# nosnoc/LCQPow

Measured on AMD Instinct MI355X. Metric: LCQPs/sec (batched dense n=256,nC=512,nComp=64), higher is better.
Workload: dtype f64; 1 GPU; synthetic dense batch=1024/GPU n=256 nC=512 nComp=64 (BASELINE configs[2]; SplitMix64 seed0=0x4C43515000000001, perturbStep=0, printLevel=NONE); global_batch=1024, parallelism=batch-sharded x1, no collective, solved=1024

## Files before the change

include/lcqp_hip.h:

```cpp
#ifndef LCQP_HIP_H
#define LCQP_HIP_H

#include <stddef.h>
#include <stdint.h>

#ifdef __cplusplus
extern "C" {
#endif

#define LCQP_SUCCESSFUL_RETURN 0
#define LCQP_INVALID_ARGUMENT 100
#define LCQP_INVALID_OBJECTIVE_LINEAR_TERM 116
#define LCQP_INVALID_CONSTRAINT_MATRIX 117
#define LCQP_INVALID_COMPLEMENTARITY_MATRIX 118
#define LCQP_INVALID_LOWER_COMPLEMENTARITY_BOUND 120
#define LCQP_MAX_ITERATIONS_REACHED 200
#define LCQP_MAX_PENALTY_REACHED 201
#define LCQP_SUBPROBLEM_SOLVER_ERROR 203
#define LCQP_LCQPOBJECT_NOT_SETUP 300
#define LCQP_HIP_ERROR 900
#define LCQP_HIP_UNSUPPORTED 901

typedef struct {
    double complementarityTolerance;
// ... 106 lines not shown
                                           const double* R, const double* A, void* stream);
int  lcqp_hip_batch_get_solution_device(lcqp_hip_batch_t* b, double* x, double* y, lcqp_stats_t* stats, void* stream);
int  lcqp_hip_batch_sensitivity_device(lcqp_hip_batch_t* b, int blocked, int nrhs, const double* v,
                                       double* dg, double* db, int* side, int* info, void* stream);
int  lcqp_hip_batch_adjoint_device(lcqp_hip_batch_t* b, const double* vx, const double* vy,
                                   double* dg, double* db, int* side, int* info,
                                   int reduce, double* dQ, double* dA, double* dL, double* dR, void* stream);
int  lcqp_hip_batch_adjoint_blocked_device(lcqp_hip_batch_t* b, int nrhs, const double* vx, const double* vy,
                                           double* dg, double* db, int* side, int* info, void* stream);
int  lcqp_hip_batch_jacobian_device(lcqp_hip_batch_t* b, int first, int count, double* Jg, double* Jb, int* side, int* info, void* stream);
int  lcqp_hip_batch_jacobian_duals_device(lcqp_hip_batch_t* b, int first, int count, double* Jyg, double* Jyb, int* side, int* info, void* stream);

int  lcqp_hip_batch_get_trace(lcqp_hip_batch_t* b, int instance, int cap, double* scalars, double* x, int* len);
int  lcqp_hip_batch_read_profile(lcqp_hip_batch_t* b, unsigned long long* out);
void* lcqp_hip_batch_stream(lcqp_hip_batch_t* b);
double lcqp_hip_batch_algorithmic_bytes(lcqp_hip_batch_t* b);
int    lcqp_hip_batch_work_sums(lcqp_hip_batch_t* b, double out[6]);

int lcqp_hip_util_symv(int batch, int n, double alpha, const double* A, const double* b, const double* c, double* d);
int lcqp_hip_util_gemv_t(int batch, int m, int n, const double* A, const double* b, double* c);
int lcqp_hip_util_gemv(int batch, int m, int n, const double* A, const double* b, double* c);
int lcqp_hip_util_rows_list(int batch, int m, int n, const double* A, const int* list, int nlist, const double* x, const double* coef,
                            double* dots, double* outT);
int lcqp_hip_util_symm_product(int batch, int m, int n, const double* A, const double* B, double* C);
typedef struct lcqp_hip_csc lcqp_hip_csc_t;
lcqp_hip_csc_t* lcqp_hip_csc_create(int m, int n, int nnz, const int* p, const int* i, const double* x, int device);
void lcqp_hip_csc_destroy(lcqp_hip_csc_t* M);
int lcqp_hip_csc_apply(lcqp_hip_csc_t* M, int transposed, double alpha, const double* b, const double* c, double* d,
                       int repeat, float* ms);
int lcqp_hip_bench_rows(int batch, int m, int n, int mode, int repeat, float* ms);
int lcqp_hip_chol_solve(int batch, int n, const double* K, const double* b, double* x, int repeat, float* ms);


typedef struct lcqp_hip_sparse lcqp_hip_sparse_t;
lcqp_hip_sparse_t* lcqp_hip_sparse_create(int batch, int nV, int nC, int nComp, const int* Qp, const int* Qi,
                                          const int* Ap, const int* Ai, int device);
void lcqp_hip_sparse_destroy(lcqp_hip_sparse_t* s);
const char* lcqp_hip_sparse_last_error(void);
int  lcqp_hip_sparse_sched_profile(lcqp_hip_sparse_t* s, unsigned long long* out21);
int  lcqp_hip_sparse_bandwidth(const lcqp_hip_sparse_t* s);
int  lcqp_hip_sparse_lanes(const lcqp_hip_sparse_t* s);
int  lcqp_hip_sparse_fronts(const lcqp_hip_sparse_t* s);
int  lcqp_hip_sparse_general_ordering(const lcqp_hip_sparse_t* s);
int  lcqp_hip_sparse_border(const lcqp_hip_sparse_t* s);
int  lcqp_hip_sparse_get_ordering(const lcqp_hip_sparse_t* s, int* perm);
int  lcqp_hip_sparse_set_options(lcqp_hip_sparse_t* s, const lcqp_options_t* opt);
// ... 69 lines not shown
```

lcqpow_amd/__init__.py:

```python
from .capi import (Options, Stats, BatchLCQP, BatchPipeline, SubsolverHIP, default_options, lib, library_path, request_hw_queues, solve_mixed,
                   util_symv, util_gemv, util_gemv_t, util_symm_product, util_rows_list, chol_solve, device_count, CSCMatrix, SparseBatchLCQP,
                   split_bound_derivatives)
```

lcqpow_amd/capi.py:

```python
import contextlib
import ctypes as C
import os
import sys

import numpy as np

_HERE = os.path.dirname(os.path.abspath(__file__))
_SO = os.environ.get("LCQPOW_HIP_LIBRARY") or os.path.join(_HERE, "liblcqpow_hip.so")
c_double_p = C.POINTER(C.c_double)

SEED0 = 0x4C43515000000001
SUCCESSFUL_RETURN = 0
SUBPROBLEM_SOLVER_ERROR = 203
MAX_ITERATIONS_REACHED = 200
MAX_PENALTY_REACHED = 201


class Options(C.Structure):
    _fields_ = [
        ("complementarityTolerance", C.c_double), ("stationarityTolerance", C.c_double),
        ("initialPenaltyParameter", C.c_double), ("penaltyUpdateFactor", C.c_double),
        ("maxPenaltyParameter", C.c_double), ("etaDynamicPenalty", C.c_double),
        ("solveZeroPenaltyFirst", C.c_int), ("perturbStep", C.c_int), ("maxIterations", C.c_int),
        ("nDynamicPenalty", C.c_int), ("printLevel", C.c_int), ("storeSteps", C.c_int),
# ... 882 lines not shown
    _check(lib().lcqp_hip_util_gemv(batch, m, n, _p(A), _p(b), _p(c)), "util_gemv")
    return c


def util_gemv_t(A, b):
    A = _arr(A); b = _arr(b)
    batch, m, n = A.shape
    c = np.zeros((batch, n))
    _check(lib().lcqp_hip_util_gemv_t(batch, m, n, _p(A), _p(b), _p(c)), "util_gemv_t")
    return c


def util_rows_list(A, lists, x=None, coef=None, dots0=None):
    A = _arr(A); x = _arr(x); coef = _arr(coef)
    batch, m, n = A.shape
    lists = np.ascontiguousarray(lists, dtype=np.int32)
    dots = np.zeros((batch, m)) if dots0 is None else np.ascontiguousarray(dots0, dtype=np.float64).copy()
    out = np.zeros((batch, n))
    _check(lib().lcqp_hip_util_rows_list(batch, m, n, _p(A), lists.ctypes.data_as(C.POINTER(C.c_int)), lists.shape[1], _p(x), _p(coef),
                                         _p(dots) if x is not None else None, _p(out) if coef is not None else None), "util_rows_list")
    return dots, out


def util_symm_product(A, B):
    A = _arr(A); B = _arr(B)
    batch, m, n = A.shape
    Cm = np.zeros((batch, n, n))
    _check(lib().lcqp_hip_util_symm_product(batch, m, n, _p(A), _p(B), _p(Cm)), "util_symm_product")
    return Cm


def chol_solve(K, b, repeat=1):
    K = _arr(K); b = _arr(b)
    batch, n = K.shape[0], K.shape[1]
    x = np.zeros((batch, n)); ms = C.c_float(0)
    _check(lib().lcqp_hip_chol_solve(batch, n, _p(K), _p(b), _p(x), repeat, C.byref(ms)), "chol_solve")
    return x, ms.value


class CSCMatrix:

    def __init__(self, m, n, p, i, x, device=0):
        self.m, self.n = m, n
        p = np.ascontiguousarray(p, dtype=np.int32); i = np.ascontiguousarray(i, dtype=np.int32); x = _arr(x)
        ip = C.POINTER(C.c_int)
        self.h = lib().lcqp_hip_csc_create(m, n, len(x), p.ctypes.data_as(ip), i.ctypes.data_as(ip), _p(x), device)
# ... 207 lines not shown
```

lcqpow_amd/csrc/lcqp_dev.hpp:

```cpp
#pragma once
#include "lcqp_wg.hpp"
#include "../../include/lcqp_hip.h"

namespace lcqp {

enum { V_G, V_GPHI, V_GTIL, V_XK, V_PK, V_XNEW, V_GK, V_QX, V_CX, V_QP, V_CP, V_STATK, V_TMP,
       V_XQ, V_XA, V_XT, V_R1, V_C, V_DU, V_W, V_RHS, V_LB, V_UB, V_X0, V_R1S, V_GS, V_ATY, V_QXN, V_XS, V_XREF, V_NUM };
enum { M_L, M_U, M_RHOV, M_YQ, M_YA, M_ZA, M_YT, M_EX, M_COEF, M_EXS, M_DY, M_RN, M_MG, M_YLV, M_HOTV, M_NUM };
enum { I_ST, I_STT, I_DEP, I_PRIO, I_SLOT, I_LIST, I_LIST2, I_HOTC, I_NUM };
enum { S_R2, S_DY, S_D0, S_SV, S_W, S_NUM };

struct InstInfo {
    int mE, nfin, hasY0, setupFail, haveSolution, isSetup, nT, prioCtr;
    int ndep, ns;
    int cNnz, kReady, rnReady, nHot;
    double scale, sigma, spv, rhoAdmm, phiConst;
    int warm, pad0;
    double rho0;
    double hist[64];
    double work[6];
};

struct DevBatch {
    int B, n, np, nC, nComp, mA, boxcap, mEcap, capS, nblk, nd;
// ... 49 lines not shown
    c.E = db.E + (size_t)b * db.mEcap * np; c.Et = db.Et + (size_t)b * db.mEcap * np;
    c.F1 = db.F1 + (size_t)b * np * np; c.FK = db.FK + (size_t)b * np * np;
    c.S = db.S + (size_t)b * db.capS * db.capS;
    c.MM = db.MM + (size_t)b * db.mMld * db.mMld;
    c.S2 = db.S2 + (size_t)b * db.capS * db.capS; c.DS = db.DS + (size_t)b * (db.capS / 64) * 4096;
    c.crow = db.crow + (size_t)b * db.capS;
    c.D1 = db.D1 + (size_t)b * db.nblk * 4096; c.dscr = db.dscr + (size_t)b * 4096;
    c.nv = db.nv + (size_t)b * V_NUM * np; c.mv = db.mv + (size_t)b * M_NUM * db.mEcap;
    c.sv = db.sv + (size_t)b * S_NUM * db.capS;
    c.mi = db.mi + (size_t)b * I_NUM * db.mEcap; c.idx = db.idx + (size_t)b * db.capS;
    c.boxidx = db.boxidx + (size_t)b * np;
    c.info = db.info + b;
    c.mE = uniform_i(c.info->mE);
    c.lds = lds;
    c.cAdmm = c.cTrials = c.cFact = c.cCorr = c.cSweeps = 0;
#ifdef LCQP_PROFILE
    for (int k = 0; k < 16; k++) c.prof[k] = 0;
    c.tlast = clock64();
#endif
    return c;
}

enum { P_LCQP = 0, P_RESID = 1, P_GRAM = 2, P_CHOL = 3, P_CORR_L1 = 4, P_CORR_ROWS = 5, P_CORR_S = 6, P_ADMM = 7, P_MISC = 8, P_DEL = 9, P_UPD_PRE = 10 };
#if defined(LCQP_PROFILE) && !defined(LCQP_PROFILE_BULK)
#define PROF(c, k) do { unsigned long long t_ = clock64(); (c).prof[k] += t_ - (c).tlast; (c).tlast = t_; } while (0)
#else
#define PROF(c, k) do { } while (0)
#endif
#if defined(LCQP_PROFILE) && defined(LCQP_PROFILE_BULK)
#define PROFB0(c) do { (c).tlast = clock64(); } while (0)
#define PROFB(c, k) do { unsigned long long t_ = clock64(); (c).prof[k] += t_ - (c).tlast; (c).tlast = t_; } while (0)
#else
#define PROFB0(c) do { } while (0)
#define PROFB(c, k) do { } while (0)
#endif

__device__ __forceinline__ double clipd(double v, double lo, double hi) { return v < lo ? lo : (v > hi ? hi : v); }

template <int NCH>
__device__ __forceinline__ void qp_admm(Ctx<NCH>& c, const double* g, int n_it)
{
    constexpr int np = 128 * NCH;
    const lcqp_options_t& o = c.db->opt;
    const int t = tid_here(), mE = c.mE;
    const double alpha = o.admmAlpha, sigma = c.info->sigma;
    double *xa = c.V(V_XA), *rhs = c.V(V_RHS), *w = c.V(V_W);
    double *ya = c.M(M_YA), *za = c.M(M_ZA), *rhov = c.M(M_RHOV), *coef = c.M(M_COEF), *ex = c.M(M_EX), *dyl = c.M(M_DY);
    const double *l = c.M(M_L), *u = c.M(M_U);
    PROF(c, P_MISC);
    for (int it = 0; it < n_it; it++) {
        const int t = tid_here();
        for (int r = t; r < mE; r += WG) coef[r] = rhov[r] * za[r] - ya[r];
        __syncthreads();
        wg_rows<NCH>(c.E, nullptr, mE, nullptr, nullptr, coef, c.lds,
                     [&](int i, double s) { rhs[i] = sigma * xa[i] - g[i] + s; });
        wg_trsv<wg_ncopy(NCH) == 2>(c.FK, np, c.nblk, rhs, true, c.lds);
        wg_trsv<wg_ncopy(NCH) == 2>(c.FK, np, c.nblk, rhs, false, c.lds);
// ... 546 lines not shown
    int* hotc = c.I(I_HOTC);
    const double* hotv = c.M(M_HOTV);
    const double *l = c.M(M_L), *u = c.M(M_U);
    int *dep = c.I(I_DEP), *prio = c.I(I_PRIO), *list = c.I(I_LIST), *rslot = c.I(I_SLOT);
    double *r2 = c.Sv(S_R2), *dy = c.Sv(S_DY);
    int* idx = c.idx;
    const double shrinkF = uniform_d(1.0 + 1e-6 + o.feasTol);
    int na = 0, nsl = 0, fact_valid = 0;
    int prioCtr = uniform_i(c.info->prioCtr);
    const int capNa = min(min(min(max(2 * c.n, 64), mE), capS), max_active(NCH));

    double xnrm = 0.0;
    int capOn = 0;
    int nrefine = 0;
    const int maxTrials = damp ? o.maxTrials + 4 * c.n + 32 : o.maxTrials;
    const PolishView v = {x, r1, cv, du, qx, xs, xref, yt, ex, mg, st, ylv, rn, hotc, hotv, l, u, dep, prio, list, rslot, r2, dy, idx,
                          g, ytol, rtolG, reuse, damp, spv, shrinkF, capNa, maxTrials};
    for (int trial = 0; trial < maxTrials; trial++) {
        const int t = tid_here();
        c.cTrials++;
        int changed = 0, nlv = 0, have_true = 0, need_true = 0;
        const bool cold = (trial == 0 && !reuse);
        PROF(c, P_MISC);
        if (trial == 0) {
            if (reuse) {
                const double *r1s = c.V(V_R1S), *gs0 = c.V(V_GS), *exs = c.M(M_EXS);
                for (int i = t; i < np; i += WG) r1[i] = (r1s[i] + (gs0[i] - g[i])) - spv * (x[i] - xref[i]);
                wg_map<4>(mE, [&](int r) { return exs[r]; }, [&](int r, double v) { ex[r] = v; });
                __syncthreads();
                have_true = 1;
            } else {
                if (!uniform_i(c.info->rnReady)) {
                    wg_row_norms<NCH>(c.E, mE, rn, hotc, c.M(M_HOTV));
                    int nh = 0;
                    for (int r = t; r < mE; r += WG) nh += (hotc[r] >= 0);
                    nh = block_sum_i(nh, c.lds);
                    if (t == 0) { c.info->rnReady = 1; c.info->nHot = nh; }
                }
                int cntA = 0;
                wg_map<4>(mE, [&](int r) { return MapID{st[r], yt[r]}; },
                          [&](int r, MapID v) { if (v.s == ST_INACT && v.a != 0.0) yt[r] = 0.0; ylv[r] = 0.0; cntA += (v.s != ST_INACT); });
                capOn = (block_sum_i(cntA, c.lds) == 0);
                (void)polish_sweep_distance<NCH>(c, v, xnrm);
                need_true = 1;
            }
        } else {
            const double dl = polish_sweep_distance<NCH>(c, v, xnrm);
            int cntLv = 0;
            int rLeave = -1;
            if (damp) rLeave = polish_damped_leave_row(st, yt, mE, ytol, t, c.lds);
            wg_map<4>(mE, [&](int r) { return MapID3{st[r], yt[r], mg[r], rn[r]}; },
                      [&](int r, MapID3 v) {
                          int s = v.s;
                          if (((s == ST_LOWER && v.a > ytol) || (s == ST_UPPER && v.a < -ytol)) && (!damp || r == rLeave)) { ylv[r] = v.a; yt[r] = 0.0; st[r] = ST_INACT; s = ST_INACT; cntLv++; }
                          mg[r] = (s != ST_INACT) ? -1.0 : v.b - v.c * dl;
                      });
            nlv = block_sum_i(cntLv, c.lds);
            changed = nlv > 0;
            const bool depRows = uniform_i(c.info->ndep) > 0;
            const int nread = wg_compact(mE, [&](int r) { return (st[r] == ST_INACT) ? !(mg[r] > 1e-10) : (depRows && dep[r] != 0); }, list, c.lds);
            wg_rows<NCH, true>(c.E, list, nread, x, ex, nullptr, c.lds, [](int, double) {}, hotc, hotv);
            double vcut = 0.0;
            int rEnter = -1;
            if (damp) {
                vcut = INFINITY;
                if (!changed) {
                    double vm = 0.0;
                    for (int a = t; a < nread; a += WG) vm = fmax(vm, polish_violation(v, o, list[a]));
                    vm = block_max(vm, c.lds);
                    if (vm > 0.0) {
                        int rb = 1 << 30;
                        for (int a = t; a < nread; a += WG) { const int r = list[a]; if (polish_violation(v, o, r) >= vm) rb = min(rb, r); }
                        rEnter = (int)(-block_max((double)(-rb), c.lds) + 0.5);
                        vcut = vm;
                    }
                }
            } else
            if (capOn) {
                double vm = 0.0, cv = 0.0, vmax, nviol;
                for (int a = t; a < nread; a += WG) { const double vi = polish_violation(v, o, list[a]); if (vi > 0.0) { cv += 1.0; vm = fmax(vm, vi); } }
                block_max_sum(vm, cv, vmax, nviol, c.lds);
                const int cap = max(c.n / 8, 16);
                if (nviol > (double)cap) {
                    double lo = 0.0, hi = vmax;
// ... 14 lines not shown
                const double e = ex[r], ftol = o.feasTol * (1.0 + fabs(e));
                if (s == ST_INACT) {
                    const bool may = !damp || r == rEnter;
                    if (may && e < l[r] - ftol && l[r] - e >= vcut) { st[r] = ST_LOWER; chg |= 1; }
                    else if (may && e > u[r] + ftol && e - u[r] >= vcut) { st[r] = ST_UPPER; chg |= 1; }
                    else mg[r] = fmin(e - (l[r] - ftol), (u[r] + ftol) - e);
                } else if (depRows && dep[r]) {
                    bool viol, inside = false;
                    if (s == ST_LOWER) { viol = e < l[r] - ftol; inside = e > l[r] + ftol; }
                    else if (s == ST_UPPER) { viol = e > u[r] + ftol; inside = e < u[r] - ftol; }
                    else viol = fabs(e - l[r]) > ftol;
                    if (inside) { const double yv = yt[r]; ylv[r] = yv; yt[r] = 0.0; st[r] = ST_INACT; cntLv2 += (yv != 0.0); chg |= 1; }
                    else if (viol) { prio[r] = prioCtr + 1; chg |= 2; }
                }
            }
            if (depRows) nlv += block_sum_i(cntLv2, c.lds);
            const bool countDense = mE <= 4000;
            const unsigned packed = (unsigned)block_sum_i((chg & 1) | (((chg >> 1) & 1) << 10) | ((countDense ? nDense : 0) << 20), c.lds);
            const int chgBits = ((packed & 1023u) ? 1 : 0) | (((packed >> 10) & 1023u) ? 2 : 0);
            if (t == 0) c.info->work[4] += countDense ? (double)(packed >> 20) : (double)nread;
            if (chgBits & 2) { prioCtr++; if (t == 0) c.info->prioCtr = prioCtr; }
            changed |= (chgBits != 0);
            need_true = !changed;
        }
        PROF(c, P_RESID);
        if (need_true) {
            int* lact = c.I(I_LIST2);
            wg_symv<NCH>(c.Q, nullptr, c.n, x, nullptr, qx, nullptr, nullptr, nullptr, c.lds);
            const int nact = wg_compact(mE, [&](int r) { return cold || st[r] != ST_INACT; }, lact, c.lds);
            wg_rows<NCH, true>(c.E, lact, nact, x, ex, yt, c.lds, [&](int i, double s) { const double ro = -g[i] - qx[i] - s; du[i] = ro; r1[i] = ro - spv * (x[i] - xref[i]); cv[i] = fabs(g[i]) + fabs(qx[i]) + fabs(s); }, hotc, hotv);
            c.cSweeps++;
            if (cold) {
                if (t == 0) c.info->work[4] += (double)(nact - uniform_i(c.info->nHot));
                wg_map<4>(mE, [&](int r) { return MapID3{st[r], ex[r], l[r], u[r]}; },
                          [&](int r, MapID3 v) {
                              const double e = v.a, ftol = o.feasTol * (1.0 + fabs(e));
                              mg[r] = (v.s != ST_INACT) ? -1.0 : fmin(e - (v.b - ftol), (v.c + ftol) - e);
                          });
                __syncthreads();
            } else {
                double res_stat, rscale;
                wg_maxabs2(r1, cv, np, c.n, res_stat, rscale, c.lds);
                const double rtolS = uniform_d(fmax(rtolG, 64.0 * 2.221e-16 * rscale));
                double res_eq = 0.0, bmax = 0.0, nDense2 = 0.0;
                for (int a = t; a < nact; a += WG) {
                    const int r = lact[a];
                    const int s = st[r];
                    nDense2 += (hotc[r] < 0) ? 1.0 : 0.0;
                    if (s == ST_INACT) continue;
                    const double bb = (s == ST_UPPER) ? u[r] : l[r];
                    const double rr = fabs(bb - ex[r]);
                    const bool above = rr > 16.0 * 2.221e-16 * (fabs(bb) + rn[r] * xnrm);
                    if (above) res_eq = fmax(res_eq, rr);
                    bmax = fmax(bmax, fabs(bb));
                    if (rslot[r] >= 0 && above) nDense2 += 1048576.0;
                }
                int nloose;
                { double re, nd; block_max_sum(res_eq, nDense2, re, nd, c.lds); res_eq = re; nloose = (int)(nd * (1.0 / 1048576.0)); nd -= 1048576.0 * nloose; if (t == 0) c.info->work[4] += nd; }
                bmax = block_max(bmax, c.lds);
#ifdef LCQP_TRACE_QP
                if (tid_here() == 0) printf("  hip trial %d stage 2: res_stat %.3e (tol %.3e) res_eq %.3e (tol %.3e) loose %d scale %.2e |x| %.2e\n", trial, res_stat, rtolS, res_eq, o.resTol * (1.0 + bmax), nloose, rscale, xnrm);
#endif
                if (res_stat <= rtolS && res_eq <= o.resTol * (1.0 + bmax) && nloose > 0 && nrefine < 2 && trial + 1 < maxTrials) {
                    nrefine++;
                } else
                if (res_stat <= rtolS && res_eq <= o.resTol * (1.0 + bmax) && !(wg_maxabs(du, np, c.lds) <= rtolS)) {
                    for (int i = t; i < np; i += WG) { xref[i] = x[i]; r1[i] = du[i]; }
                    __syncthreads();
                } else
                if (res_stat <= rtolS && res_eq <= o.resTol * (1.0 + bmax)) {
                    double *r1s = c.V(V_R1S), *gs0 = c.V(V_GS), *exs = c.M(M_EXS), *aty = c.V(V_ATY);
                    double* qxn = c.V(V_QXN);
                    for (int i = t; i < np; i += WG) { const double ro = du[i]; r1s[i] = ro; gs0[i] = g[i]; aty[i] = g[i] + qx[i] + ro; qxn[i] = qx[i]; }
                    wg_map<4>(mE, [&](int r) { return ex[r]; }, [&](int r, double v) { exs[r] = v; });
                    __syncthreads();
                    PROF(c, P_RESID);
                    return 1;
                }
            }
            have_true = 1;
            PROF(c, P_RESID);
        }
        if (changed) fact_valid = 0;
        if (!fact_valid) {
            int nT = uniform_i(c.info->nT), ns = uniform_i(c.info->ns);
            int touched = 0, ndepNow = 0;
            const int ndel = wg_compact(ns, [&](int sl) { const int r = idx[sl]; return r >= 0 && st[r] == ST_INACT; }, list, c.lds);
            int cntAdd = 0;
            wg_map<4>(mE, [&](int r) { return MapID{st[r], (double)rslot[r]}; }, [&](int, MapID v) { cntAdd += (v.s != ST_INACT && v.a < 0.0); });
            const int nadd = block_sum_i(cntAdd, c.lds);
            if (trial >= 2 && nT - ndel + nadd > c.n && ndel + nadd > max(c.n / 2, 32)) { polish_give_up<NCH>(c, v); return 0; }
            PROF(c, P_UPD_PRE);
            const bool bulk = prioCtr > 0 || (nT == 0 && nadd > 0) || (ndel > 0 && ndel >= max(nT / 2, 8)) || nadd >= 16 || (3 * ndel + 7 * nadd >= 96);
            int naAll = 0;
            if (bulk) {
                int cntAct = 0;
                for (int r = t; r < mE; r += WG) cntAct += (st[r] != ST_INACT);
                naAll = block_sum_i(cntAct, c.lds);
                ti_reset<NCH>(c, nT, ns);
            }
            if (bulk && naAll <= capNa) {
                int na2 = 0;
                for (int stamp = prioCtr; stamp >= 1; stamp--)
                    na2 += wg_compact(mE, [&](int r) { return st[r] != ST_INACT && prio[r] == stamp; }, idx + na2, c.lds);
// ... 501 lines not shown
```

lcqpow_amd/csrc/lcqp_hip_util.hip:

```cpp
#include "lcqp_hip_batch.hpp"
#include "../../include/lcqp_synth.h"

#include <algorithm>
#include <cstring>
#include <memory>
#include <vector>

using namespace lcqp;
using namespace lcqp_rt;

__global__ __launch_bounds__(WG) void k_chol(int np, int nblk, int n, double* F, double* dscr, int* fail)
{
    LCQP_LDS
    const int b = blockIdx.x;
    wg_chol(F + (size_t)b * np * np, np, nblk, n, 0.0, dscr + (size_t)b * 4096, nullptr, fail + b, lds, 0);
}

__global__ __launch_bounds__(WG, 4) void k_backsolve(int np, int nblk, const double* F, const double* rhs, double* x)
{
    LCQP_LDS
    const int b = blockIdx.x;
    double* xv = x + (size_t)b * np;
    for (int i = threadIdx.x; i < np; i += WG) xv[i] = rhs[(size_t)b * np + i];
    __syncthreads();
// ... 79 lines not shown

extern "C" int lcqp_hip_util_rows_list(int batch, int m, int n, const double* A, const int* list, int nlist, const double* x, const double* coef,
                                       double* dots, double* outT)
{ return guarded(dense_err(), [&] {
    if (n <= 0 || n > 4096 || batch <= 0 || m <= 0 || nlist < 0 || nlist > m || !list) return LCQP_HIP_UNSUPPORTED;
    const SizeKernels* k = dense_kernels(padded_nch(n));
    if (!k) return LCQP_HIP_UNSUPPORTED;
    const int np = 128 * k->nch;
    DevMem tb;
    double *dA, *dx = nullptr, *dd = nullptr, *dcf = nullptr, *dout = nullptr;
    int* dl;
    if (!tb.alloc(dense_err(), dA, (size_t)batch * m * np) || (x && !tb.alloc(dense_err(), dx, (size_t)batch * np)) ||
        (dots && !tb.alloc(dense_err(), dd, (size_t)batch * m, dots)) ||
        (coef && !tb.alloc(dense_err(), dcf, (size_t)batch * m, coef)) || (outT && !tb.alloc(dense_err(), dout, (size_t)batch * np)) ||
        !tb.alloc(dense_err(), dl, (size_t)batch * nlist, list))
        return LCQP_HIP_ERROR;
    int rc = upload_padded(dA, A, batch, m, n, np, m); if (rc) return rc;
    if (x) { rc = upload_padded(dx, x, batch, 1, n, np, 1); if (rc) return rc; }
    k->util_rows_list(batch, 0, m, nlist, dA, dl, dx, dd, dcf, dout);
    HIPCHK(dense_err(), hipDeviceSynchronize());
    if (dots) HIPCHK(dense_err(), hipMemcpy(dots, dd, sizeof(double) * (size_t)batch * m, hipMemcpyDeviceToHost));
    if (outT) return download_padded(outT, dout, batch, 1, n, np, 1);
    return 0;
}); }

extern "C" int lcqp_hip_util_gemv(int batch, int m, int n, const double* A, const double* b, double* c)
{
    return guarded(dense_err(), [&] { return util_rows(batch, m, n, A, b, c, nullptr, nullptr); });
}
extern "C" int lcqp_hip_util_gemv_t(int batch, int m, int n, const double* A, const double* b, double* c)
{
    return guarded(dense_err(), [&] { return util_rows(batch, m, n, A, nullptr, nullptr, b, c); });
}

extern "C" int lcqp_hip_util_symm_product(int batch, int m, int n, const double* A, const double* Bm, double* C)
{ return guarded(dense_err(), [&] {
    lcqp_hip_batch* h = lcqp_hip_batch_create(batch, n, 0, m, 0, 0);
    if (!h) return LCQP_HIP_ERROR;
    DevBatch& d = h->db;
    int rc = upload_padded(d.E, A, batch, m, n, d.np, d.mEcap);
    if (!rc) {
        std::vector<double> buf((size_t)d.mEcap * d.np);
        for (int b = 0; b < batch && !rc; b++) {
            if (hipMemcpy(buf.data(), d.E + (size_t)b * d.mEcap * d.np, sizeof(double) * buf.size(), hipMemcpyDeviceToHost) != hipSuccess) { rc = LCQP_HIP_ERROR; break; }
            for (int r = 0; r < m; r++) memcpy(&buf[(size_t)(m + r) * d.np], Bm + ((size_t)b * m + r) * n, sizeof(double) * n);
            if (hipMemcpy(d.E + (size_t)b * d.mEcap * d.np, buf.data(), sizeof(double) * buf.size(), hipMemcpyHostToDevice) != hipSuccess) rc = LCQP_HIP_ERROR;
// ... 194 lines not shown
```

lcqpow_amd/csrc/lcqp_kernels.hpp:

```cpp
#pragma once
#include "lcqp_dev.hpp"
#include "lcqp_launch.hpp"
#include "../../include/lcqp_synth.h"

using namespace lcqp;


template <int NCH>
__device__ __forceinline__ double prepare_vectors(const DevBatch& db, Ctx<NCH>& c, Lds lds, double scale)
{
    constexpr int np = 128 * NCH;
    const int b = c.b, t = threadIdx.x;
    const int mA = db.mA, nC = db.nC, nComp = db.nComp;
    const int nfin = c.info->nfin;
    const int mE = mA + nfin;
    double *l = c.M(M_L), *u = c.M(M_U), *rhov = c.M(M_RHOV);
    for (int k = t; k < nfin; k += WG) {
        const int bi = c.boxidx[k];
        l[mA + k] = c.V(V_LB)[bi]; u[mA + k] = c.V(V_UB)[bi];
    }
    __syncthreads();
    const double rho = db.opt.admmRho * scale;
    for (int r = t; r < mE; r += WG) {
        const double lo = l[r], hi = u[r];
// ... 1083 lines not shown
template <int NCH>
__global__ __launch_bounds__(WG) void k_util_rows(int m, const double* A, const double* x, double* dots, const double* coef, double* outT)
{
    LCQP_LDS_N(NCH)
    constexpr int np = 128 * NCH;
    const int b = blockIdx.x;
    double* o = outT ? outT + (size_t)b * np : nullptr;
    wg_rows<NCH>(A + (size_t)b * m * np, nullptr, m, x ? x + (size_t)b * np : nullptr, dots ? dots + (size_t)b * m : nullptr,
                 coef ? coef + (size_t)b * m : nullptr, lds, [&](int i, double s) { if (o) o[i] = s; });
}

template <int NCH>
__global__ __launch_bounds__(WG) void k_util_rows_list(int m, int nlist, const double* A, const int* list, const double* x, double* dots, const double* coef, double* outT)
{
    LCQP_LDS_N(NCH)
    constexpr int np = 128 * NCH;
    const int b = blockIdx.x;
    double* o = outT ? outT + (size_t)b * np : nullptr;
    wg_rows<NCH, true>(A + (size_t)b * m * np, list + (size_t)b * nlist, nlist, x ? x + (size_t)b * np : nullptr, dots ? dots + (size_t)b * m : nullptr,
                       coef ? coef + (size_t)b * m : nullptr, lds, [&](int i, double s) { if (o) o[i] = s; });
}

template <int NCH>
static void launch_run(const DevBatch& db, int grid, hipStream_t s)
{
    if constexpr (NCH <= 2) {
        static_assert(6 * 128 * NCH <= LDS_ROWS_OFF, "k_lcqp_run<NCH, true>: the sweeps' scratch must end below the row state");
        if (db.mEcap <= LDS_ROWS_MAX && 4 * db.capS <= LDS_ROWS_OFF) { hipLaunchKernelGGL((k_lcqp_run<NCH, true, LCQP_VARIANT>), dim3(grid), dim3(WG), 0, s, db); return; }
    }
    hipLaunchKernelGGL((k_lcqp_run<NCH, false, LCQP_VARIANT>), dim3(grid), dim3(WG), 0, s, db);
}

template <int NCH>
static void launch_qp_solve(const DevBatch& db, int grid, hipStream_t s, int initial)
{
    hipLaunchKernelGGL((k_qp_solve<NCH, LCQP_VARIANT>), dim3(grid), dim3(WG), 0, s, db, initial);
}

namespace lcqp {
#ifdef LCQP_TU_FEW
template <int NCH>
const RunKernels& few_kernels()
{
    static const RunKernels k = {launch_run<NCH>, launch_qp_solve<NCH>};
    return k;
}
// ... 23 lines not shown
        };
        t.sensitivity_dual = [](const DevBatch& db, int grid, hipStream_t s, int nrhs, const double* v, const double* vy, double* dg, double* dbo, int* side, int* sinfo) {
            hipLaunchKernelGGL((k_sensitivity<NCH, true>), dim3(grid), dim3(WG), 0, s, db, nrhs, v, dg, dbo, side, sinfo, vy);
        };
        t.build_C = [](const DevBatch& db, int grid, hipStream_t s) { hipLaunchKernelGGL((k_build_C<NCH>), dim3(grid), dim3(WG), 0, s, db); };
        t.compress_C = [](const DevBatch& db, int grid, hipStream_t s) { hipLaunchKernelGGL((k_compress_C<NCH>), dim3(grid), dim3(WG), 0, s, db); };
        t.factor = [](const DevBatch& db, int grid, hipStream_t s) { hipLaunchKernelGGL((k_factor<NCH, 1>), dim3(grid), dim3(WG), 0, s, db); };
        t.factor_full = [](const DevBatch& db, int grid, hipStream_t s) { hipLaunchKernelGGL((k_factor<NCH, NCH <= 2 ? 4 : 1>), dim3(grid), dim3(WG), 0, s, db); };
        t.trsm = [](const DevBatch& db, int grid, hipStream_t s) { hipLaunchKernelGGL((k_trsm<NCH>), dim3(grid), dim3(WG), 0, s, db); };
        t.trsm_streamed = [](const DevBatch& db, int grid, hipStream_t s) { hipLaunchKernelGGL((k_trsm_streamed<NCH>), dim3(grid), dim3(WG), 0, s, db); };
        t.build_M = [](const DevBatch& db, int grid, hipStream_t s) { hipLaunchKernelGGL((k_build_M<NCH>), dim3(grid), dim3(WG), 0, s, db); };
        t.run = {launch_run<NCH>, launch_qp_solve<NCH>};
        t.synth_fill = [](const DevBatch& db, int grid, hipStream_t s, uint64_t seed0, uint64_t first) { hipLaunchKernelGGL((k_synth_fill<NCH>), dim3(grid), dim3(WG), 0, s, db, seed0, first); };
        t.synth_Q = [](const DevBatch& db, int grid, hipStream_t s) { hipLaunchKernelGGL((k_synth_Q<NCH>), dim3(grid), dim3(WG), 0, s, db); };
        t.util_symv = [](int grid, hipStream_t s, int n, double alpha, const double* A, const double* b, const double* c, double* d) {
            hipLaunchKernelGGL((k_util_symv<NCH>), dim3(grid), dim3(WG), 0, s, n, alpha, A, b, c, d);
        };
        t.util_rows = [](int grid, hipStream_t s, int m, const double* A, const double* x, double* dots, const double* coef, double* outT) {
            hipLaunchKernelGGL((k_util_rows<NCH>), dim3(grid), dim3(WG), 0, s, m, A, x, dots, coef, outT);
        };
        t.util_rows_list = [](int grid, hipStream_t s, int m, int nlist, const double* A, const int* list, const double* x, double* dots, const double* coef, double* outT) {
            hipLaunchKernelGGL((k_util_rows_list<NCH>), dim3(grid), dim3(WG), 0, s, m, nlist, A, list, x, dots, coef, outT);
        };
        return t;
    }();
    return k;
}
#endif
}
```

lcqpow_amd/csrc/lcqp_launch.hpp:

```cpp
#pragma once
#include "lcqp_dev.hpp"

namespace lcqp {
#pragma GCC visibility push(hidden)

struct RunKernels {
    void (*lcqp_run)(const DevBatch& db, int grid, hipStream_t s);
    void (*qp_solve)(const DevBatch& db, int grid, hipStream_t s, int initial);
};

using BatchKernel = void (*)(const DevBatch& db, int grid, hipStream_t s);

struct SizeKernels {
    int nch;
    RunKernels run;
    const RunKernels* few;
    BatchKernel prepare;
    void (*refresh)(const DevBatch& db, int grid, hipStream_t s, int mode, const double* rho0);
    void (*prepare_warm)(const DevBatch& db, int grid, hipStream_t s, const double* rho0);
    BatchKernel build_C, compress_C;
    BatchKernel factor, factor_full;
    BatchKernel trsm, trsm_streamed, build_M;
    void (*synth_fill)(const DevBatch& db, int grid, hipStream_t s, uint64_t seed0, uint64_t first);
    BatchKernel synth_Q;
    void (*sensitivity)(const DevBatch& db, int grid, hipStream_t s, int nrhs, const double* v, double* dg, double* dbo, int* side, int* sinfo);
    void (*sensitivity_dual)(const DevBatch& db, int grid, hipStream_t s, int nrhs, const double* v, const double* vy, double* dg, double* dbo, int* side, int* sinfo);
    void (*sensitivity_blk)(const DevBatch& db, int grid, hipStream_t s, int first, int nrhs, const double* v, double* dg, double* dbo, int* side, int* sinfo);
    void (*sensitivity_blk_dual)(const DevBatch& db, int grid, hipStream_t s, int first, int nrhs, const double* v, const double* vy, int unit,
                                 double* dg, double* dbo, int* side, int* sinfo, int* rowpos);
    void (*util_symv)(int grid, hipStream_t s, int n, double alpha, const double* A, const double* b, const double* c, double* d);
    void (*util_rows)(int grid, hipStream_t s, int m, const double* A, const double* x, double* dots, const double* coef, double* outT);
    void (*util_rows_list)(int grid, hipStream_t s, int m, int nlist, const double* A, const int* list, const double* x, double* dots, const double* coef, double* outT);
};

template <int NCH> const SizeKernels& size_kernels();
template <int NCH> const RunKernels& few_kernels();

#pragma GCC visibility pop
}
```

lcqpow_amd/csrc/lcqp_wg.hpp:

```cpp
#pragma once
#include <hip/hip_runtime.h>
#include <stdint.h>

namespace lcqp {

constexpr int WG = 256;
constexpr int NWAVE = 4;
constexpr int wg_ncopy(int nch) { return nch > 16 ? 2 : 4; }
constexpr int arena_doubles(int nch) { return (wg_ncopy(nch) + 2) * 128 * nch > 4512 ? (wg_ncopy(nch) + 2) * 128 * nch : 4512; }
constexpr int ARENA = arena_doubles(4);
constexpr int TILE_LD = 65;
constexpr int max_active(int nch) { return 64 * (arena_doubles(nch) / (5 * 64)); }
constexpr int LCQP_MAX_ACTIVE = max_active(4);

enum { ST_INACT = 0, ST_LOWER = 1, ST_UPPER = 2, ST_EQ = 3 };

constexpr int LDS_ROWS_MAX = 640;
constexpr int LDS_ROWS_OFF = 2048;
static_assert(LDS_ROWS_OFF + 3 * LDS_ROWS_MAX + LDS_ROWS_MAX / 2 <= 4512, "row state must fit the arena");

struct Lds {
    double* arena;
    double* red;
    int* ired;
// ... 382 lines not shown
                }
            }
#pragma unroll
            for (int d = 0; d < D; d++) {
                if (x) {
                    double dsum = 0.0;
#pragma unroll
                    for (int k = 0; k < NCH; k++) dsum += mm[d][k].x * xr[2 * k] + mm[d][k].y * xr[2 * k + 1];
                    dsum = wave_sum(dsum);
                    if (l == j0 + d) mydot = dsum;
                }
                if (coef && cfs[d] != 0.0) {
#pragma unroll
                    for (int k = 0; k < NCH; k++) { acc[2 * k] += cfs[d] * mm[d][k].x; acc[2 * k + 1] += cfs[d] * mm[d][k].y; }
                }
            }
        }
        if (mine && dots && (!BYROW || myrow >= 0)) dots[BYROW ? myrow : mya] = mydot;
    }
    if (coef) wg_combine<NCH>(acc, lds, post);
    else __syncthreads();
}

template <bool TWO = false>
__device__ __forceinline__ void wg_trsv(const double* __restrict__ F, int ld, int nblk, double* vec, bool forward, Lds lds)
{
    const int nn = 64 * nblk;
    double* b = lds.arena;
    double* red = lds.arena + nn;
    for (int i = tid_here(); i < nn; i += WG) b[i] = vec[i];
    __syncthreads();
    const int l = lane_id(), w = wave_id();
    for (int s = 0; s < nblk; s++) {
        const int I = forward ? s : nblk - 1 - s;
        {
            const double* Fd = F + (size_t)(64 * I) * ld + 64 * I;
            double f[16];
#pragma unroll
            for (int cc = 0; cc < 16; cc++) {
                const int c = 16 * w + cc;
                f[cc] = 0.0;
                if (forward ? (c <= l) : (c >= l)) f[cc] = ld_stream(Fd + (size_t)c * ld + l);
            }
            double acc = 0.0;
#pragma unroll
            for (int cc = 0; cc < 16; cc++) {
// ... 350 lines not shown
```

Baseline: 31010 LCQPs/s.

## Fuse Q symv with active-row E products in the residual stage

Adds a fused device routine that streams Q rows and the active E rows in one pass, producing Qx, E^T y and the row dots together with one shared LDS reduction instead of separate symv and row passes. It is used for small padded sizes (NCH<=2, which covers n=256), while larger sizes keep the old two-call path. The leaving-row check is also switched to a dots-only routine that skips the combine reduction. A test utility and residual-stage profiling macros are added as well. This trades extra registers and a larger LDS footprint (eight partial copies) for fewer barriers and passes.

```diff
diff --git a/include/lcqp_hip.h b/include/lcqp_hip.h
--- a/include/lcqp_hip.h
+++ b/include/lcqp_hip.h
@@ -152,6 +152,8 @@
 int lcqp_hip_util_gemv(int batch, int m, int n, const double* A, const double* b, double* c);
 int lcqp_hip_util_rows_list(int batch, int m, int n, const double* A, const int* list, int nlist, const double* x, const double* coef,
                             double* dots, double* outT);
+int lcqp_hip_util_symv_rows(int batch, int n, int m, const double* Q, const double* E, const int* list, int nlist, const double* x, const double* coef,
+                            int use_hot, int two_pass, double* qx, double* ety, double* dots);
 int lcqp_hip_util_symm_product(int batch, int m, int n, const double* A, const double* B, double* C);
 typedef struct lcqp_hip_csc lcqp_hip_csc_t;
 lcqp_hip_csc_t* lcqp_hip_csc_create(int m, int n, int nnz, const int* p, const int* i, const double* x, int device);
diff --git a/lcqpow_amd/__init__.py b/lcqpow_amd/__init__.py
--- a/lcqpow_amd/__init__.py
+++ b/lcqpow_amd/__init__.py
@@ -1,3 +1,3 @@
 from .capi import (Options, Stats, BatchLCQP, BatchPipeline, SubsolverHIP, default_options, lib, library_path, request_hw_queues, solve_mixed,
-                   util_symv, util_gemv, util_gemv_t, util_symm_product, util_rows_list, chol_solve, device_count, CSCMatrix, SparseBatchLCQP,
+                   util_symv, util_gemv, util_gemv_t, util_symm_product, util_rows_list, util_symv_rows, chol_solve, device_count, CSCMatrix, SparseBatchLCQP,
                    split_bound_derivatives)
diff --git a/lcqpow_amd/capi.py b/lcqpow_amd/capi.py
--- a/lcqpow_amd/capi.py
+++ b/lcqpow_amd/capi.py
@@ -928,6 +928,19 @@
     return dots, out
 
 
+def util_symv_rows(Q, E, lists, x, coef, use_hot=False, two_pass=False, dots0=None):
+    Q = _arr(Q); E = _arr(E); x = _arr(x); coef = _arr(coef)
+    batch, m, n = E.shape
+    lists = np.ascontiguousarray(lists, dtype=np.int32).reshape(batch, -1)
+    dots = np.zeros((batch, m)) if dots0 is None else np.ascontiguousarray(dots0, dtype=np.float64).copy()
+    qx, ety = np.zeros((batch, n)), np.zeros((batch, n))
+    f = lib().lcqp_hip_util_symv_rows
+    f.argtypes = [C.c_int, C.c_int, C.c_int, c_double_p, c_double_p, C.POINTER(C.c_int), C.c_int, c_double_p, c_double_p, C.c_int, C.c_int] + [c_double_p] * 3
+    _check(f(batch, n, m, _p(Q), _p(E), lists.ctypes.data_as(C.POINTER(C.c_int)), lists.shape[1], _p(x), _p(coef), int(use_hot), int(two_pass),
+             _p(qx), _p(ety), _p(dots)), "util_symv_rows")
+    return qx, ety, dots
+
+
 def util_symm_product(A, B):
     A = _arr(A); B = _arr(B)
     batch, m, n = A.shape
diff --git a/lcqpow_amd/csrc/lcqp_dev.hpp b/lcqpow_amd/csrc/lcqp_dev.hpp
--- a/lcqpow_amd/csrc/lcqp_dev.hpp
+++ b/lcqpow_amd/csrc/lcqp_dev.hpp
@@ -95,7 +95,7 @@
 }
 
 enum { P_LCQP = 0, P_RESID = 1, P_GRAM = 2, P_CHOL = 3, P_CORR_L1 = 4, P_CORR_ROWS = 5, P_CORR_S = 6, P_ADMM = 7, P_MISC = 8, P_DEL = 9, P_UPD_PRE = 10 };
-#if defined(LCQP_PROFILE) && !defined(LCQP_PROFILE_BULK)
+#if defined(LCQP_PROFILE) && !defined(LCQP_PROFILE_BULK) && !defined(LCQP_PROFILE_RESID)
 #define PROF(c, k) do { unsigned long long t_ = clock64(); (c).prof[k] += t_ - (c).tlast; (c).tlast = t_; } while (0)
 #else
 #define PROF(c, k) do { } while (0)
@@ -106,6 +106,14 @@
 #else
 #define PROFB0(c) do { } while (0)
 #define PROFB(c, k) do { } while (0)
+#endif
+enum { R_ENTRY = 0, R_A = 1, R_B = 2, R_Q = 3, R_COMPACT = 4, R_E = 5, R_TAIL = 6 };
+#if defined(LCQP_PROFILE) && defined(LCQP_PROFILE_RESID)
+#define PROFR0(c) do { (c).tlast = clock64(); } while (0)
+#define PROFR(c, k) do { unsigned long long t_ = clock64(); (c).prof[k] += t_ - (c).tlast; (c).tlast = t_; } while (0)
+#else
+#define PROFR0(c) do { } while (0)
+#define PROFR(c, k) do { } while (0)
 #endif
 
 __device__ __forceinline__ double clipd(double v, double lo, double hi) { return v < lo ? lo : (v > hi ? hi : v); }
@@ -698,6 +706,7 @@
         int changed = 0, nlv = 0, have_true = 0, need_true = 0;
         const bool cold = (trial == 0 && !reuse);
         PROF(c, P_MISC);
+        PROFR0(c);
         if (trial == 0) {
             if (reuse) {
                 const double *r1s = c.V(V_R1S), *gs0 = c.V(V_GS), *exs = c.M(M_EXS);
@@ -720,6 +729,7 @@
                 (void)polish_sweep_distance<NCH>(c, v, xnrm);
                 need_true = 1;
             }
+            PROFR(c, R_ENTRY);
         } else {
             const double dl = polish_sweep_distance<NCH>(c, v, xnrm);
             int cntLv = 0;
@@ -733,9 +743,10 @@
                       });
             nlv = block_sum_i(cntLv, c.lds);
             changed = nlv > 0;
+            PROFR(c, R_A);
             const bool depRows = uniform_i(c.info->ndep) > 0;
             const int nread = wg_compact(mE, [&](int r) { return (st[r] == ST_INACT) ? !(mg[r] > 1e-10) : (depRows && dep[r] != 0); }, list, c.lds);
-            wg_rows<NCH, true>(c.E, list, nread, x, ex, nullptr, c.lds, [](int, double) {}, hotc, hotv);
+            wg_row_dots<NCH>(c.E, list, nread, x, ex, hotc, hotv);
             double vcut = 0.0;
             int rEnter = -1;
             if (damp) {
@@ -796,13 +807,15 @@
             if (chgBits & 2) { prioCtr++; if (t == 0) c.info->prioCtr = prioCtr; }
             changed |= (chgBits != 0);
             need_true = !changed;
+            PROFR(c, R_B);
         }
         PROF(c, P_RESID);
         if (need_true) {
             int* lact = c.I(I_LIST2);
-            wg_symv<NCH>(c.Q, nullptr, c.n, x, nullptr, qx, nullptr, nullptr, nullptr, c.lds);
             const int nact = wg_compact(mE, [&](int r) { return cold || st[r] != ST_INACT; }, lact, c.lds);
-            wg_rows<NCH, true>(c.E, lact, nact, x, ex, yt, c.lds, [&](int i, double s) { const double ro = -g[i] - qx[i] - s; du[i] = ro; r1[i] = ro - spv * (x[i] - xref[i]); cv[i] = fabs(g[i]) + fabs(qx[i]) + fabs(s); }, hotc, hotv);
+            PROFR(c, R_COMPACT);
+            wg_resid_stream<NCH>(c.Q, c.n, c.E, lact, nact, x, qx, ex, yt, c.lds, [&](int i, double q, double s) { const double ro = -g[i] - q - s; du[i] = ro; r1[i] = ro - spv * (x[i] - xref[i]); cv[i] = fabs(g[i]) + fabs(q) + fabs(s); }, hotc, hotv);
+            PROFR(c, R_Q);
             c.cSweeps++;
             if (cold) {
                 if (t == 0) c.info->work[4] += (double)(nact - uniform_i(c.info->nHot));
@@ -849,11 +862,13 @@
                     wg_map<4>(mE, [&](int r) { return ex[r]; }, [&](int r, double v) { exs[r] = v; });
                     __syncthreads();
                     PROF(c, P_RESID);
+                    PROFR(c, R_TAIL);
                     return 1;
                 }
             }
             have_true = 1;
             PROF(c, P_RESID);
+            PROFR(c, R_TAIL);
         }
         if (changed) fact_valid = 0;
         if (!fact_valid) {
diff --git a/lcqpow_amd/csrc/lcqp_hip_util.hip b/lcqpow_amd/csrc/lcqp_hip_util.hip
--- a/lcqpow_amd/csrc/lcqp_hip_util.hip
+++ b/lcqpow_amd/csrc/lcqp_hip_util.hip
@@ -125,6 +125,33 @@
     if (dots) HIPCHK(dense_err(), hipMemcpy(dots, dd, sizeof(double) * (size_t)batch * m, hipMemcpyDeviceToHost));
     if (outT) return download_padded(outT, dout, batch, 1, n, np, 1);
     return 0;
+}); }
+
+extern "C" int lcqp_hip_util_symv_rows(int batch, int n, int m, const double* Q, const double* E, const int* list, int nlist, const double* x, const double* coef,
+                                       int use_hot, int two_pass, double* qx, double* ety, double* dots)
+{ return guarded(dense_err(), [&] {
+    if (n <= 0 || n > 4096 || batch <= 0 || m <= 0 || nlist < 0 || nlist > m || !Q || !E || !list || !x || !coef || !qx || !ety || !dots) return LCQP_HIP_UNSUPPORTED;
+    for (size_t i = 0; i < (size_t)batch * nlist; i++) if (list[i] < 0 || list[i] >= m) return LCQP_HIP_UNSUPPORTED;
+    const SizeKernels* k = dense_kernels(padded_nch(n));
+    if (!k) return LCQP_HIP_UNSUPPORTED;
+    const int np = 128 * k->nch;
+    DevMem tb;
+    double *dQ, *dE, *dx, *dcf, *dd, *dq, *dout, *drn, *dhv;
+    int *dl, *dhc;
+    if (!tb.alloc(dense_err(), dQ, (size_t)batch * np * np) || !tb.alloc(dense_err(), dE, (size_t)batch * m * np) || !tb.alloc(dense_err(), dx, (size_t)batch * np) ||
+        !tb.alloc(dense_err(), dcf, (size_t)batch * m, coef) || !tb.alloc(dense_err(), dd, (size_t)batch * m, dots) ||
+        !tb.alloc(dense_err(), dq, (size_t)batch * np) || !tb.alloc(dense_err(), dout, (size_t)batch * np) || !tb.alloc(dense_err(), drn, (size_t)batch * m) ||
+        !tb.alloc(dense_err(), dhv, (size_t)batch * m) || !tb.alloc(dense_err(), dhc, (size_t)batch * m) || !tb.alloc(dense_err(), dl, (size_t)batch * (nlist > 0 ? nlist : 1)))
+        return LCQP_HIP_ERROR;
+    if (nlist > 0) HIPCHK(dense_err(), hipMemcpy(dl, list, sizeof(int) * (size_t)batch * nlist, hipMemcpyHostToDevice));
+    int rc = upload_padded(dQ, Q, batch, n, n, np, np); if (rc) return rc;
+    rc = upload_padded(dE, E, batch, m, n, np, m); if (rc) return rc;
+    rc = upload_padded(dx, x, batch, 1, n, np, 1); if (rc) return rc;
+    k->util_symv_rows(batch, 0, n, m, nlist, dQ, dE, dl, dx, dcf, use_hot, two_pass, drn, dhc, dhv, dq, dout, dd);
+    HIPCHK(dense_err(), hipDeviceSynchronize());
+    HIPCHK(dense_err(), hipMemcpy(dots, dd, sizeof(double) * (size_t)batch * m, hipMemcpyDeviceToHost));
+    rc = download_padded(qx, dq, batch, 1, n, np, 1); if (rc) return rc;
+    return download_padded(ety, dout, batch, 1, n, np, 1);
 }); }
 
 extern "C" int lcqp_hip_util_gemv(int batch, int m, int n, const double* A, const double* b, double* c)
diff --git a/lcqpow_amd/csrc/lcqp_kernels.hpp b/lcqpow_amd/csrc/lcqp_kernels.hpp
--- a/lcqpow_amd/csrc/lcqp_kernels.hpp
+++ b/lcqpow_amd/csrc/lcqp_kernels.hpp
@@ -1129,6 +1129,30 @@
 }
 
 template <int NCH>
+__global__ __launch_bounds__(WG) void k_util_symv_rows(int n, int m, int nlist, const double* Q, const double* E, const int* list, const double* x, const double* coef,
+                                                       int useHot, int twoPass, double* rn, int* hotc, double* hotv, double* qx, double* ety, double* dots)
+{
+    LCQP_LDS_N(NCH)
+    constexpr int np = 128 * NCH;
+    const int b = blockIdx.x;
+    const double *Eb = E + (size_t)b * m * np, *Qb = Q + (size_t)b * np * np, *xb = x + (size_t)b * np, *cf = coef + (size_t)b * m;
+    const int* lb = list + (size_t)b * nlist;
+    int* hc = hotc + (size_t)b * m;
+    double *hv = hotv + (size_t)b * m, *q = qx + (size_t)b * np, *o = ety + (size_t)b * np, *dt = dots + (size_t)b * m;
+    if (useHot) wg_row_norms<NCH>(Eb, m, rn + (size_t)b * m, hc, hv);
+    else { for (int r = threadIdx.x; r < m; r += WG) { hc[r] = -1; hv[r] = 0.0; } __syncthreads(); }
+    if (twoPass == 2) {
+        wg_symv<NCH>(Qb, nullptr, n, xb, nullptr, q, nullptr, nullptr, nullptr, lds);
+        wg_row_dots<NCH>(Eb, lb, nlist, xb, dt, hc, hv);
+        wg_rows<NCH, true>(Eb, lb, nlist, nullptr, nullptr, cf, lds, [&](int i, double s) { o[i] = s; }, hc, hv);
+    } else if (twoPass) {
+        wg_symv<NCH>(Qb, nullptr, n, xb, nullptr, q, nullptr, nullptr, nullptr, lds);
+        wg_rows<NCH, true>(Eb, lb, nlist, xb, dt, cf, lds, [&](int i, double s) { o[i] = s; }, hc, hv);
+    } else
+        wg_resid_stream<NCH>(Qb, n, Eb, lb, nlist, xb, q, dt, cf, lds, [&](int i, double, double s) { o[i] = s; }, hc, hv);
+}
+
+template <int NCH>
 static void launch_run(const DevBatch& db, int grid, hipStream_t s)
 {
     if constexpr (NCH <= 2) {
@@ -1198,6 +1222,10 @@
         t.util_rows_list = [](int grid, hipStream_t s, int m, int nlist, const double* A, const int* list, const double* x, double* dots, const double* coef, double* outT) {
             hipLaunchKernelGGL((k_util_rows_list<NCH>), dim3(grid), dim3(WG), 0, s, m, nlist, A, list, x, dots, coef, outT);
         };
+        t.util_symv_rows = [](int grid, hipStream_t s, int n, int m, int nlist, const double* Q, const double* E, const int* list, const double* x, const double* coef,
+                              int useHot, int twoPass, double* rn, int* hotc, double* hotv, double* qx, double* ety, double* dots) {
+            hipLaunchKernelGGL((k_util_symv_rows<NCH>), dim3(grid), dim3(WG), 0, s, n, m, nlist, Q, E, list, x, coef, useHot, twoPass, rn, hotc, hotv, qx, ety, dots);
+        };
         return t;
     }();
     return k;
diff --git a/lcqpow_amd/csrc/lcqp_launch.hpp b/lcqpow_amd/csrc/lcqp_launch.hpp
--- a/lcqpow_amd/csrc/lcqp_launch.hpp
+++ b/lcqpow_amd/csrc/lcqp_launch.hpp
@@ -31,6 +31,8 @@
     void (*util_symv)(int grid, hipStream_t s, int n, double alpha, const double* A, const double* b, const double* c, double* d);
     void (*util_rows)(int grid, hipStream_t s, int m, const double* A, const double* x, double* dots, const double* coef, double* outT);
     void (*util_rows_list)(int grid, hipStream_t s, int m, int nlist, const double* A, const int* list, const double* x, double* dots, const double* coef, double* outT);
+    void (*util_symv_rows)(int grid, hipStream_t s, int n, int m, int nlist, const double* Q, const double* E, const int* list, const double* x, const double* coef,
+                           int useHot, int twoPass, double* rn, int* hotc, double* hotv, double* qx, double* ety, double* dots);
 };
 
 template <int NCH> const SizeKernels& size_kernels();
diff --git a/lcqpow_amd/csrc/lcqp_wg.hpp b/lcqpow_amd/csrc/lcqp_wg.hpp
--- a/lcqpow_amd/csrc/lcqp_wg.hpp
+++ b/lcqpow_amd/csrc/lcqp_wg.hpp
@@ -428,6 +428,190 @@
     else __syncthreads();
 }
 
+template <int NCH, class Post>
+__device__ __forceinline__ void wg_symv_rows(const double* __restrict__ Q, int n, const double* __restrict__ Mx, const int* __restrict__ idx, int m,
+                        const double* __restrict__ x, double* dots, const double* __restrict__ coef, Lds lds, Post post,
+                        const int* __restrict__ hotc, const double* __restrict__ hotv)
+{
+    constexpr int np = 128 * NCH;
+    static_assert(NCH <= 2, "wg_symv_rows: a lane holds one x entry of its wave's rows of Q (np / 4 <= 64)");
+    static_assert(wg_ncopy(NCH) == 4 && 8 * np <= LDS_ROWS_OFF, "wg_symv_rows: two sets of four partial copies must end below the row state");
+    constexpr int D = ROWS_IN_FLIGHT;
+    const int l = lane_id(), w = wave_id();
+    const int nchunk = (m + 15) >> 4;
+    int myrow = -1, myhc = -1;
+    double mycoef = 0.0, myhv = 0.0;
+    if (w < nchunk) {
+        const int mya = (w << 4) + l;
+        if (l < 16 && mya < m) myrow = idx[mya];
+        if (myrow >= 0) { mycoef = coef[myrow]; myhc = hotc[myrow]; myhv = hotv[myrow]; }
+    }
+    double xr[2 * NCH], aq[2 * NCH], acc[2 * NCH];
+#pragma unroll
+    for (int k = 0; k < NCH; k++) {
+        const double2 xv = reinterpret_cast<const double2*>(x)[64 * k + l];
+        xr[2 * k] = xv.x; xr[2 * k + 1] = xv.y;
+        aq[2 * k] = aq[2 * k + 1] = acc[2 * k] = acc[2 * k + 1] = 0.0;
+    }
+    const int rq = w + NWAVE * l;
+    const double xq = (rq < n) ? x[rq] : 0.0;
+    const int nR = min(np, ((n + NWAVE * D - 1) / (NWAVE * D)) * (NWAVE * D));
+    for (int r0 = w, j0 = 0; r0 < nR; r0 += NWAVE * D, j0 += D) {
+        double2 m0[D][NCH];
+#pragma unroll
+        for (int d = 0; d < D; d++) {
+            const double2* row0 = reinterpret_cast<const double2*>(Q + (size_t)(r0 + NWAVE * d) * np) + l;
+#pragma unroll
+            for (int k = 0; k < NCH; k++) m0[d][k] = ld_stream(row0 + 64 * k);
+        }
+#pragma unroll
+        for (int d = 0; d < D; d++) {
+            const double x0 = wave_bcast(xq, (j0 + d) & 63);
+#pragma unroll
+            for (int k = 0; k < NCH; k++) { aq[2 * k] += m0[d][k].x * x0; aq[2 * k + 1] += m0[d][k].y * x0; }
+        }
+    }
+    for (int ch = w; ch < nchunk; ch += NWAVE) {
+        const int a0 = ch << 4;
+        const int mya = a0 + l;
+        const bool mine = (l < 16) && (mya < m);
+        if (ch != w) {
+            myrow = mine ? idx[mya] : -1;
+            mycoef = 0.0; myhc = -1; myhv = 0.0;
+            if (myrow >= 0) { mycoef = coef[myrow]; myhc = hotc[myrow]; myhv = hotv[myrow]; }
+        }
+        double mydot = 0.0;
+        const int cnt = min(16, m - a0);
+        for (int j0 = 0; j0 < cnt; j0 += D) {
+            double2 mm[D][NCH];
+            double cfs[D];
+#pragma unroll
+            for (int d = 0; d < D; d++) {
+                const int row = wave_bcast_i(myrow, (j0 + d) & 63);
+                cfs[d] = wave_bcast(mycoef, (j0 + d) & 63);
+                const int hc = wave_bcast_i(myhc, (j0 + d) & 63);
+                if (hc >= 0) {
+                    const double hv = wave_bcast(myhv, (j0 + d) & 63);
+#pragma unroll
+                    for (int k = 0; k < NCH; k++) {
+                        mm[d][k] = double2{0.0, 0.0};
+                        if ((hc >> 7) == k && ((hc & 127) >> 1) == l) { if (hc & 1) mm[d][k].y = hv; else mm[d][k].x = hv; }
+                    }
+                } else if (row >= 0) {
+                    const double2* rp = reinterpret_cast<const double2*>(Mx + (size_t)row * np) + l;
+#pragma unroll
+                    for (int k = 0; k < NCH; k++) mm[d][k] = ld_stream(rp + 64 * k);
+                } else {
+#pragma unroll
+                    for (int k = 0; k < NCH; k++) mm[d][k] = double2{0.0, 0.0};
+                }
+            }
+#pragma unroll
+            for (int d = 0; d < D; d++) {
+                double dsum = 0.0;
+#pragma unroll
+                for (int k = 0; k < NCH; k++) dsum += mm[d][k].x * xr[2 * k] + mm[d][k].y * xr[2 * k + 1];
+                dsum = wave_sum(dsum);
+                if (l == j0 + d) mydot = dsum;
+                if (cfs[d] != 0.0) {
+#pragma unroll
+                    for (int k = 0; k < NCH; k++) { acc[2 * k] += cfs[d] * mm[d][k].x; acc[2 * k + 1] += cfs[d] * mm[d][k].y; }
+                }
+            }
+        }
+        if (mine && myrow >= 0) dots[myrow] = mydot;
+    }
+    double* red = lds.arena;
+#pragma unroll
+    for (int k = 0; k < NCH; k++) {
+        red[w * np + 128 * k + 2 * l] = aq[2 * k];
+        red[w * np + 128 * k + 2 * l + 1] = aq[2 * k + 1];
+        red[(4 + w) * np + 128 * k + 2 * l] = acc[2 * k];
+        red[(4 + w) * np + 128 * k + 2 * l + 1] = acc[2 * k + 1];
+    }
+    __syncthreads();
+    for (int c = tid_here(); c < np; c += WG)
+        post(c, red[c] + red[np + c] + red[2 * np + c] + red[3 * np + c], red[4 * np + c] + red[5 * np + c] + red[6 * np + c] + red[7 * np + c]);
+    __syncthreads();
+}
+
+template <int NCH>
+__device__ __forceinline__ void wg_row_dots(const double* __restrict__ Mx, const int* __restrict__ idx, int m, const double* __restrict__ x, double* dots,
+                        const int* __restrict__ hotc, const double* __restrict__ hotv)
+{
+    constexpr int np = 128 * NCH;
+    constexpr int D = (NCH > 8) ? 1 : (NCH == 4 ? 2 : ROWS_IN_FLIGHT);
+    const int l = lane_id(), w = wave_id();
+    const int nchunk = (m + 15) >> 4;
+    if (w < nchunk) {
+        double xr[2 * NCH];
+#pragma unroll
+        for (int k = 0; k < NCH; k++) {
+            const double2 xv = reinterpret_cast<const double2*>(x)[64 * k + l];
+            xr[2 * k] = xv.x; xr[2 * k + 1] = xv.y;
+        }
+        for (int ch = w; ch < nchunk; ch += NWAVE) {
+            const int a0 = ch << 4;
+            const int mya = a0 + l;
+            const bool mine = (l < 16) && (mya < m);
+            const int myrow = mine ? idx[mya] : -1;
+            int myhc = -1;
+            double myhv = 0.0;
+            if (myrow >= 0) { myhc = hotc[myrow]; myhv = hotv[myrow]; }
+            double mydot = 0.0;
+            const int cnt = min(16, m - a0);
+            for (int j0 = 0; j0 < cnt; j0 += D) {
+                double2 mm[D][NCH];
+#pragma unroll
+                for (int d = 0; d < D; d++) {
+                    const int row = wave_bcast_i(myrow, (j0 + d) & 63);
+                    const int hc = wave_bcast_i(myhc, (j0 + d) & 63);
+                    if (hc >= 0) {
+                        const double hv = wave_bcast(myhv, (j0 + d) & 63);
+#pragma unroll
+                        for (int k = 0; k < NCH; k++) {
+                            mm[d][k] = double2{0.0, 0.0};
+                            if ((hc >> 7) == k && ((hc & 127) >> 1) == l) { if (hc & 1) mm[d][k].y = hv; else mm[d][k].x = hv; }
+                        }
+                    } else if (row >= 0) {
+                        const double2* rp = reinterpret_cast<const double2*>(Mx + (size_t)row * np) + l;
+#pragma unroll
+                        for (int k = 0; k < NCH; k++) mm[d][k] = ld_stream(rp + 64 * k);
+                    } else {
+#pragma unroll
+                        for (int k = 0; k < NCH; k++) mm[d][k] = double2{0.0, 0.0};
+                    }
+                }
+#pragma unroll
+                for (int d = 0; d < D; d++) {
+                    double dsum = 0.0;
+#pragma unroll
+                    for (int k = 0; k < NCH; k++) dsum += mm[d][k].x * xr[2 * k] + mm[d][k].y * xr[2 * k + 1];
+                    dsum = wave_sum(dsum);
+                    if (l == j0 + d) mydot = dsum;
+                }
+            }
+            if (mine && myrow >= 0) dots[myrow] = mydot;
+        }
+    }
+    __syncthreads();
+}
+
+constexpr bool resid_one_stream(int nch) { return nch <= 2; }
+
+template <int NCH, class Post>
+__device__ __forceinline__ void wg_resid_stream(const double* __restrict__ Q, int n, const double* __restrict__ Mx, const int* __restrict__ idx, int m,
+                        const double* __restrict__ x, double* qx, double* dots, const double* __restrict__ coef, Lds lds, Post post,
+                        const int* __restrict__ hotc, const double* __restrict__ hotv)
+{
+    if constexpr (resid_one_stream(NCH)) {
+        wg_symv_rows<NCH>(Q, n, Mx, idx, m, x, dots, coef, lds, [&](int c, double sq, double se) { qx[c] = sq; post(c, sq, se); }, hotc, hotv);
+    } else {
+        wg_symv<NCH>(Q, nullptr, n, x, nullptr, qx, nullptr, nullptr, nullptr, lds);
+        wg_rows<NCH, true>(Mx, idx, m, x, dots, coef, lds, [&](int c, double se) { post(c, qx[c], se); }, hotc, hotv);
+    }
+}
+
 template <bool TWO = false>
 __device__ __forceinline__ void wg_trsv(const double* __restrict__ F, int ld, int nblk, double* vec, bool forward, Lds lds)
 {
```

Result: no change. 31090 LCQPs/s (median of 5 runs) (+0.3%).
